# realphongha/UDP-Pose

Hardware: AMD Instinct MI355X
Metric: images/sec HRNet-W32 256x192 (infer+decode) (higher is better)
Workload: dtype f16x2 (split fp16 hi+lo operands = 22 bits, 3 fp16 MFMAs per product, fp32 accumulate); 1 GPU; w32 256x192 f16x2 inference, batch=64 per GPU, flip-test on, DARK decode (forward on 2N images + flip fuse + udp_decode_gaussian); global_batch=64, parallelism=replicas x1 (no data-path collective), weights=seeded synthetic, BN stats calibrated (tests/golden/bn_calib_w32_gaussian.npz)

## Files before the change

udp-pose_amd/csrc/conv_ws.hip:

```cpp
#include "conv_dev.h"

namespace udp {

#ifndef UDP_WS_LATE_RES
#define UDP_WS_LATE_RES 1
#endif
#ifndef UDP_WS_FAST_EPI
#define UDP_WS_FAST_EPI 1
#endif
#ifndef UDP_WS_FAST_ADDR
#define UDP_WS_FAST_ADDR 1
#endif
#ifdef UDP_OLD_SWZ
#undef UDP_WS_FAST_ADDR
#define UDP_WS_FAST_ADDR 0
#endif
#ifndef UDP_WS_INC_STEP
#define UDP_WS_INC_STEP 1
#endif
#if !UDP_WS_FAST_ADDR
#undef UDP_WS_INC_STEP
#define UDP_WS_INC_STEP 0
#endif
template <int NB>
struct ResH2 {
  u32x4 hi[NB / 2], lo[NB / 2];
};
template <int NB>
__device__ __forceinline__ void load_res_h2(ResH2<NB>& o, __amdgpu_buffer_rsrc_t r, unsigned voff, unsigned lo_off) {
#pragma unroll
  for (int h = 0; h < NB / 2; ++h) {
    o.hi[h] = __builtin_amdgcn_raw_buffer_load_b128(r, voff + 16 * h, 0, UDP_H2_RES_AUX);
    o.lo[h] = __builtin_amdgcn_raw_buffer_load_b128(r, voff + lo_off + 16 * h, 0, UDP_H2_RES_AUX);
  }
}
template <int NB>
__device__ __forceinline__ void add_res_h2(f32x4 (&v)[NB], const ResH2<NB>& o) {
#pragma unroll
  for (int h = 0; h < NB / 2; ++h) {
#if UDP_WS_FAST_EPI
    h2_add8_fast(v[2 * h], v[2 * h + 1], o.hi[h], o.lo[h]);
#else
    h2_add8(v[2 * h], v[2 * h + 1], __builtin_bit_cast(f16x8, o.hi[h]), __builtin_bit_cast(f16x8, o.lo[h]));
#endif
  }
}

template <int KS, int STRIDE, int PB, int CP, bool NCHW, bool OUT2 = false, int HS = 0, bool NUP = true, bool XP = false>
__device__ __forceinline__ void conv_ws_body(const ConvParams& p, const int tile_id, const int cby, const int xpair = 0) {
  using T = H2;
  constexpr int CK = 32, ESZ = 2, NB = 2, NW = 4;
  constexpr int PAD = KS / 2, TAPS = KS * KS;
  extern __shared__ __attribute__((aligned(UDP_WS_INC_STEP ? 512 : 16))) unsigned char smem[];

  UDP_STAMP(0);
  const int tid = threadIdx.x;
  const int lane = tid & 63;
  const int wave = __builtin_amdgcn_readfirstlane(tid >> 6);
  const int li = lane & 15;
  const int kg = lane >> 4;
  const int cp = wave % CP, pg = wave / CP;

  int t = tile_id;
  const int tx = t % p.tiles_x;
  t /= p.tiles_x;
  const int ty = t % p.tiles_y;
  const int n0 = (t / p.tiles_y) * p.G;
  const int y0 = ty * p.R;
  const int x0 = tx * p.TW;

  const int IH = p.IH, IW = p.IW;
  const int npix_in = p.G * IH * IW;
  const int in_groups = (npix_in + 15) >> 4;
  const int in_bytes = in_groups * 16 * ROWB;
  const int stage_bytes = 2 * in_bytes;
  const int nchunks = (p.Cin + CK - 1) / CK;
  const bool ragged = (p.Cin % CK) != 0;
  const int RT = p.R * p.TW;
  const int M = p.G * RT;
  const unsigned inpb = (unsigned)p.in_pitch * ESZ * 2;
  const unsigned outpb = (unsigned)p.out_pitch * ESZ * 2, respb = (unsigned)p.res_pitch * ESZ * 2;
  const unsigned in_lo = (unsigned)p.in_pitch * ESZ;
  const unsigned out_lo = (unsigned)p.out_pitch * ESZ, res_lo = (unsigned)p.res_pitch * ESZ;

  const unsigned out_pix = (unsigned)p.N * p.Hout * p.Wout;
  const __amdgpu_buffer_rsrc_t r_in = __builtin_amdgcn_make_buffer_rsrc(
      const_cast<void*>(p.in), 0, (unsigned)p.N * p.Hin * p.Win * inpb, 0x00020000);
  const unsigned npairs = (unsigned)p.CoutPad >> 5;
  const __amdgpu_buffer_rsrc_t r_w = __builtin_amdgcn_make_buffer_rsrc(
      const_cast<void*>(p.wgt), 0, (unsigned)TAPS * nchunks * npairs * 4096u, 0x00020000);
#if UDP_WS_DBG & 32
  const bool dbg_nost = nchunks == 1;
#else
  constexpr bool dbg_nost = false;
#endif
#if UDP_WS_DBG & 64
  const bool dbg_nores = nchunks == 1;
#else
  constexpr bool dbg_nores = false;
#endif
  const __amdgpu_buffer_rsrc_t r_out = __builtin_amdgcn_make_buffer_rsrc(
      p.out, 0, (!p.out || dbg_nost) ? 0 : NCHW ? (out_pix + (unsigned)p.out_skip * p.Hout * p.Wout) * p.Cout * 4 : out_pix * outpb, 0x00020000);
  const __amdgpu_buffer_rsrc_t r_bias = __builtin_amdgcn_make_buffer_rsrc(
      const_cast<float*>(p.bias), 0, (unsigned)p.CoutPad * 4u, 0x00020000);
  const __amdgpu_buffer_rsrc_t r_res = __builtin_amdgcn_make_buffer_rsrc(
      const_cast<void*>(p.res), 0, (p.res && !dbg_nores) ? out_pix * respb : 0, 0x00020000);

  const int pair = XP ? xpair : cby * CP + cp;
  const int cwave = pair * 32;
  const int cbase = cwave + 8 * kg;
  const unsigned wvoff = (unsigned)lane * 16u;
  const unsigned wpair = (unsigned)pair * 4096u;
  constexpr int AD = UDP_WS_AD;
  f16x8 ah[AD][NB], al[AD][NB];
  const int nsteps = nchunks * TAPS;
  auto load_a_at = [&](unsigned soff, f16x8 (&h)[NB], f16x8 (&l)[NB]) __attribute__((always_inline)) {
#pragma unroll
    for (int nb = 0; nb < NB; ++nb) {
      h[nb] = __builtin_bit_cast(f16x8, __builtin_amdgcn_raw_buffer_load_b128(r_w, wvoff + 2048u * nb, soff, 0));
      l[nb] = __builtin_bit_cast(f16x8, __builtin_amdgcn_raw_buffer_load_b128(r_w, wvoff + 2048u * nb + 1024u, soff, 0));
    }
  };
  auto load_a = [&](int s, f16x8 (&h)[NB], f16x8 (&l)[NB]) __attribute__((always_inline)) {
    const int c = s / TAPS, tap = s - c * TAPS;
    load_a_at((unsigned)(tap * nchunks + c) * (npairs * 4096u) + wpair, h, l);
  };

#pragma unroll
  for (int k = 0; k < AD - 1; ++k) load_a(k < nsteps ? k : nsteps - 1, ah[k], al[k]);
  f32x4 bias[NB];
#pragma unroll
  for (int nb = 0; nb < NB; ++nb)
    bias[nb] = __builtin_bit_cast(f32x4, __builtin_amdgcn_raw_buffer_load_b128(r_bias, (unsigned)(cbase + 4 * nb) * 4u, 0, 0));

  const int srow = lane >> 2, spart = lane & 3;
  const int gy0 = y0 * STRIDE - PAD, gx0 = x0 * STRIDE - PAD;
  unsigned src_off[MAXG];
#pragma unroll
  for (int i = 0; i < MAXG; ++i) {
    unsigned off = kOobOff;
    if ((wave + NW * i) * 16 < npix_in) {
      const int row = (wave + NW * i) * 16 + srow;
      const int tmp = fdiv20(row, p.mIW);
      const int ix = row - (int)__umul24(tmp, IW);
      const int g = fdiv20(tmp, p.mIH);
      const int iy = tmp - (int)__umul24(g, IH);
      const int n = n0 + g, gy = gy0 + iy, gx = gx0 + ix;
      const bool ok = row < npix_in && n < p.N && (unsigned)gy < (unsigned)p.Hin && (unsigned)gx < (unsigned)p.Win;
      const unsigned pix = __umul24(__umul24(n, p.Hin) + gy, p.Win) + gx;
      off = ok ? pix * inpb + p.in_coff * ESZ + ((spart ^ swz<T>(row)) << 4) : kOobOff;
    }
    src_off[i] = off;
  }
  auto stage = [&](int c, unsigned char* sb) __attribute__((always_inline)) {
    const unsigned coff = (unsigned)c * (CK * ESZ);
    const bool cut = ragged && c == nchunks - 1;
    const int parts_left = (p.Cin - c * CK) / 8;
#pragma unroll
    for (int i = 0; i < MAXG; ++i) {
      const int gidx = wave + NW * i;
      if (gidx < in_groups) {
        unsigned off = src_off[i] + coff;
        if (cut && (spart ^ swz<T>(gidx * 16 + srow)) >= parts_left) off = kOobOff;
        blds16(r_in, off, sb + gidx * (16 * ROWB));
        blds16(r_in, off + in_lo, sb + in_bytes + gidx * (16 * ROWB));
      }
    }
  };

  UDP_STAMP(1);
  stage(0, smem);

  int prow[PB], opix[PB], ocrd[NCHW || NUP ? PB : 1];
#pragma unroll
  for (int i = 0; i < PB; ++i) {
    const int m0 = (pg * PB + i) * 16 + li;
    const int m = m0 < M ? m0 : M - 1;
    const int g = fdiv20(m, p.mRT);
    const int rem = m - (int)__umul24(g, RT);
    const int r = fdiv20(rem, p.mTW);
    const int x = rem - (int)__umul24(r, p.TW);
    prow[i] = (int)__umul24(__umul24(g, IH) + r * STRIDE, IW) + x * STRIDE;
#if UDP_WS_FAST_ADDR
    prow[i] = prow[i] * ROWB + (kg << 4);
#endif
    const int n = n0 + g, y = y0 + r, xo = x0 + x;
    const bool ok = m0 < M && n < p.N && y < p.Hout && xo < p.Wout && (NCHW || cbase < p.Cout);
    const unsigned pix = __umul24(__umul24(n, p.Hout) + y, p.Wout) + xo;
    opix[i] = ok ? (int)pix : -1;
    if constexpr (NCHW || NUP) ocrd[i] = ok ? (y | (xo << 10) | (n << 20)) : -1;
  }

  const float winv = __builtin_ldexpf(1.f, -p.wexp);
  f32x4 acc[PB][NB];
#pragma unroll
  for (int i = 0; i < PB; ++i)
#pragma unroll
    for (int nb = 0; nb < NB; ++nb) acc[i][nb] = f32x4{0.f, 0.f, 0.f, 0.f};

  constexpr bool LATE = UDP_WS_LATE_RES && KS == 3 && STRIDE == 1 && !NCHW && AD == 3;
  constexpr int NR = NCHW ? 0 : PB * NB;
  ResH2<NB> rres[NCHW ? 1 : PB];
  constexpr int RSPLIT = LATE && PB > 6 ? PB / 2 : PB;
  auto load_res = [&](auto I0, auto I1) __attribute__((always_inline)) {
    __builtin_amdgcn_sched_barrier(0);
    asm volatile("" ::: "memory");
#pragma unroll
    for (int i = decltype(I0)::value; i < (NCHW ? 0 : decltype(I1)::value); ++i)
      load_res_h2(rres[i], r_res, opix[i] >= 0 ? (unsigned)opix[i] * respb + (p.res_coff + cbase) * ESZ : kOobOff, res_lo);
    asm volatile("" ::: "memory");
    __builtin_amdgcn_sched_barrier(0);
  };
  if constexpr (!LATE) load_res(std::integral_constant<int, 0>{}, std::integral_constant<int, PB>{});

  UDP_STAMP(2);
  int c = 0, tap = 0;
  const unsigned char* sb = smem;
  constexpr bool INC = UDP_WS_INC_STEP && LATE;
  using lds_u8 = const __attribute__((address_space(3))) unsigned char*;
  using lds_f16x8 = const __attribute__((address_space(3))) f16x8*;
  [[maybe_unused]] const unsigned lds0 = INC ? (unsigned)(size_t)(lds_u8)smem : 0u;
  [[maybe_unused]] const unsigned a_tap = (unsigned)nchunks * (npairs * 4096u);
  [[maybe_unused]] unsigned a_next = (unsigned)(AD - 1) * a_tap + wpair;
  [[maybe_unused]] int dy = 0;
  [[maybe_unused]] unsigned row_off = 0, sb_off = lds0;
  auto step = [&](auto BUFC, auto TAILC, int s) __attribute__((always_inline)) {
    constexpr int BUF = decltype(BUFC)::value, TAIL = decltype(TAILC)::value;
#if !(UDP_WS_DBG & 1)
    if constexpr (!LATE)
      load_a(s + AD - 1 < nsteps ? s + AD - 1 : nsteps - 1, ah[(BUF + AD - 1) % AD], al[(BUF + AD - 1) % AD]);
    else if constexpr (TAIL <= 0) {
      if constexpr (INC) {
        load_a_at(a_next, ah[(BUF + AD - 1) % AD], al[(BUF + AD - 1) % AD]);
        a_next += (BUF == 0 && dy == KS - 1) ? npairs * 4096u - (unsigned)(TAPS - 1) * a_tap : a_tap;
      } else {
        load_a(s + AD - 1, ah[(BUF + AD - 1) % AD], al[(BUF + AD - 1) % AD]);
      }
    }
#endif
    if constexpr (TAIL == 0) load_res(std::integral_constant<int, 0>{}, std::integral_constant<int, RSPLIT>{});
    if constexpr (TAIL == 1 && RSPLIT < PB) load_res(std::integral_constant<int, RSPLIT>{}, std::integral_constant<int, PB>{});
    if (TAIL < 0 && (INC ? BUF == 0 && dy == 0 : tap == 0)) {
      if (c == 1) UDP_STAMP(9);
      if (c == 2) UDP_STAMP(11);
      if (c == 4) UDP_STAMP(13);
      bool refill = false;
      if constexpr (STRIDE == 2 || OUT2) refill = p.sbuf && c > 0;
      if (refill) {
        __syncthreads();
        stage(c, smem);
        asm volatile("s_waitcnt vmcnt(0)" ::: "memory");
        __syncthreads();
        sb = smem;
        if constexpr (INC) sb_off = lds0;
      } else {
        if (s == 0)
          asm volatile("s_waitcnt vmcnt(%0)" ::"n"(2 * NB + (LATE ? 0 : NR)) : "memory");
        else
          asm volatile("s_waitcnt vmcnt(%0)" ::"n"(2 * NB) : "memory");
        if (s == 0) UDP_STAMP(3);
        __syncthreads();
        if (s == 0) UDP_STAMP(4);
        if (c == 1) UDP_STAMP(10);
        if (c == 2) UDP_STAMP(12);
        if (c == 4) UDP_STAMP(14);
#if !(UDP_WS_DBG & 4)
        if (c + 1 < nchunks && !((STRIDE == 2 || OUT2) && p.sbuf)) stage(c + 1, smem + ((c + 1) & 1) * stage_bytes);
#endif
        sb = smem + (c & 1) * stage_bytes;
        if constexpr (INC) sb_off = lds0 + (unsigned)((c & 1) * stage_bytes);
      }
    }
    f16x8 a2[NB];
#pragma unroll
    for (int nb = 0; nb < NB; ++nb) a2[nb] = ah[BUF][nb] * (_Float16)0x1p-11f;
    const int tap_rows = KS == 1 ? 0 : TAIL >= 0 ? (KS - 1) * IW + TAIL : (tap / KS) * IW + tap % KS;
    f16x8 xh[3], xl[3];
#if UDP_WS_FAST_ADDR
    const unsigned tap_off = INC ? sb_off + row_off + (unsigned)(BUF * ROWB) : (unsigned)(sb - smem) + (unsigned)tap_rows * ROWB;
    auto load_b = [&](int i, f16x8& h, f16x8& l) __attribute__((always_inline)) {
      const unsigned rb = (unsigned)prow[i] + tap_off;
      const unsigned a = __builtin_amdgcn_bitop3_b32(rb >> 3, rb, 32u, 0x6c);
      if constexpr (INC) {
        h = *reinterpret_cast<lds_f16x8>((size_t)a);
        l = *reinterpret_cast<lds_f16x8>((size_t)(a + (unsigned)in_bytes));
      } else {
        const unsigned char* q = smem + a;
        h = *reinterpret_cast<const f16x8*>(q);
        l = *reinterpret_cast<const f16x8*>(q + in_bytes);
      }
    };
#else
    auto load_b = [&](int i, f16x8& h, f16x8& l) __attribute__((always_inline)) {
      const int row = prow[i] + tap_rows;
      const unsigned char* q = sb + row * ROWB + ((kg ^ swz<T>(row)) << 4);
      h = *reinterpret_cast<const f16x8*>(q);
      l = *reinterpret_cast<const f16x8*>(q + in_bytes);
    };
#endif
    load_b(0, xh[0], xl[0]);
    if (PB > 1) load_b(1, xh[1], xl[1]);
#pragma unroll
    for (int i = 0; i < PB; ++i) {
#if !(UDP_WS_DBG & 2)
      if (i + 2 < PB) load_b(i + 2, xh[(i + 2) % 3], xl[(i + 2) % 3]);
#endif
      __builtin_amdgcn_sched_barrier(0);
#if UDP_WS_DBG & 16
      acc[i][0] = __builtin_amdgcn_mfma_f32_16x16x32_f16(ah[BUF][0] + al[BUF][1] + a2[0] + a2[1], xh[i % 3] + xl[i % 3], acc[i][0], 0, 0, 0);
#else
#pragma unroll
      for (int nb = 0; nb < NB; ++nb) acc[i][nb] = __builtin_amdgcn_mfma_f32_16x16x32_f16(ah[BUF][nb], xh[i % 3], acc[i][nb], 0, 0, 0);
#pragma unroll
      for (int nb = 0; nb < NB; ++nb) acc[i][nb] = __builtin_amdgcn_mfma_f32_16x16x32_f16(al[BUF][nb], xh[i % 3], acc[i][nb], 0, 0, 0);
#pragma unroll
      for (int nb = 0; nb < NB; ++nb) acc[i][nb] = __builtin_amdgcn_mfma_f32_16x16x32_f16(a2[nb], xl[i % 3], acc[i][nb], 0, 0, 0);
#endif
    }
    if constexpr (TAIL < 0) {
      if constexpr (INC) {
        if constexpr (BUF == KS - 1) {
          ++dy;
          row_off += (unsigned)IW * ROWB;
          if (dy == KS) {
            dy = 0;
            row_off = 0;
            ++c;
          }
        }
      } else if (++tap == TAPS) {
        tap = 0;
        ++c;
      }
    }
  };
  constexpr std::integral_constant<int, -1> LOOP{};
  if constexpr (LATE) {
    for (int s = 0; s < nsteps - AD; s += AD) {
      step(std::integral_constant<int, 0>{}, LOOP, s);
      step(std::integral_constant<int, 1>{}, LOOP, s + 1);
      step(std::integral_constant<int, 2>{}, LOOP, s + 2);
    }
    step(std::integral_constant<int, 0>{}, std::integral_constant<int, 0>{}, nsteps - 3);
    step(std::integral_constant<int, 1>{}, std::integral_constant<int, 1>{}, nsteps - 2);
    step(std::integral_constant<int, 2>{}, std::integral_constant<int, 2>{}, nsteps - 1);
  } else {
    for (int s = 0; s < nsteps; s += AD) {
      step(std::integral_constant<int, 0>{}, LOOP, s);
      if (s + 1 < nsteps) step(std::integral_constant<int, 1>{}, LOOP, s + 1);
      if (s + 2 < nsteps) step(std::integral_constant<int, 2>{}, LOOP, s + 2);
      if constexpr (AD > 3) if (s + 3 < nsteps) step(std::integral_constant<int, 3>{}, LOOP, s + 3);
      if constexpr (AD > 4) if (s + 4 < nsteps) step(std::integral_constant<int, 4>{}, LOOP, s + 4);
      if constexpr (AD > 5) if (s + 5 < nsteps) step(std::integral_constant<int, 5>{}, LOOP, s + 5);
    }
  }
  UDP_STAMP(5);
#pragma unroll
  for (int i = 0; i < PB; ++i) {
#pragma unroll
    for (int nb = 0; nb < NB; ++nb)
#pragma unroll
      for (int q = 0; q < 4; ++q) acc[i][nb][q] = __builtin_fmaf(acc[i][nb][q], winv, bias[nb][q]);
    if constexpr (!NCHW) add_res_h2(acc[i], rres[i]);
  }

#if UDP_WS_FAST_EPI
  [[maybe_unused]] const float relu_lim = p.relu ? 0.f : __builtin_nanf("");
#endif
#pragma unroll
  for (int i = 0; i < PB; ++i) {
    f32x4 v[NB];
#pragma unroll
    for (int nb = 0; nb < NB; ++nb) v[nb] = acc[i][nb];
    if constexpr (NCHW) {
      const int crd = ocrd[i];
      const int y = crd & 1023, xo = (crd >> 10) & 1023, n = crd >> 20;
      const unsigned hw = __umul24(p.Hout, p.Wout);
      const int no = n >= p.flip_from ? n + p.out_skip : n;
      const unsigned base = __umul24(__umul24(__umul24(no, p.Cout), p.Hout) + y, p.Wout) + xo;
#pragma unroll
      for (int nb = 0; nb < NB; ++nb)
#pragma unroll
        for (int q = 0; q < 4; ++q) {
          const int cc = cbase + 4 * nb + q;
          float f = v[nb][q];
          if (p.relu) f = f > 0.f ? f : 0.f;
          const unsigned off = (crd >= 0 && cc < p.Cout) ? (base + cc * hw) * 4u : kOobOff;
          __builtin_amdgcn_raw_buffer_store_b32(__builtin_bit_cast(unsigned, f), r_out, off, 0, 0);
        }
    } else {
      const unsigned ooff = opix[i] >= 0 ? (unsigned)opix[i] * outpb + (p.out_coff + cbase) * ESZ : kOobOff;
      if (NUP && p.nup) {
        const int crd = ocrd[NUP ? i : 0];
        const int y = crd & 1023, xo = (crd >> 10) & 1023, n = crd >> 20;
#pragma unroll
        for (int u = 0; u < 3; ++u) {
          if (u < p.nup) {
            const int sh = p.up_shift[u];
            const long up_pix = ((long)(n * (p.Hout >> sh) + (y >> sh)) * (p.Wout >> sh) + (xo >> sh));
            if (crd >= 0)
              add_vec<T, NB>(v, reinterpret_cast<const unsigned char*>(p.up[u]) + (up_pix * p.Cout * 2 + cbase) * ESZ, p.Cout * ESZ);
          }
        }
      }
#if UDP_WS_FAST_EPI
      unsigned mag;
      if constexpr (HS) {
#pragma unroll
        for (int nb = 0; nb < NB; ++nb)
#pragma unroll
          for (int q = 0; q < 4; ++q) v[nb][q] = act_hs<HS>(v[nb][q]);
        mag = h2_mag8<false>(0u, v[0], v[1]);
      } else {
        relu8_fast(v[0], v[1], relu_lim);
        mag = p.relu ? h2_mag8<true>(0u, v[0], v[1]) : h2_mag8<false>(0u, v[0], v[1]);
      }
      h2_range_check_bits(mag);
      u32x4 shi, slo;
      h2_split8_fast(v[0], v[1], shi, slo);
      __builtin_amdgcn_raw_buffer_store_b128(shi, r_out, ooff, 0, UDP_H2_STORE_AUX);
      __builtin_amdgcn_raw_buffer_store_b128(slo, r_out, ooff + out_lo, 0, UDP_H2_STORE_AUX);
#else
      if constexpr (HS) {
#pragma unroll
        for (int nb = 0; nb < NB; ++nb)
#pragma unroll
          for (int q = 0; q < 4; ++q) v[nb][q] = act_hs<HS>(v[nb][q]);
      } else
      if (p.relu) {
#pragma unroll
        for (int nb = 0; nb < NB; ++nb)
#pragma unroll
          for (int q = 0; q < 4; ++q) v[nb][q] = v[nb][q] > 0.f ? v[nb][q] : 0.f;
      }
      store_vec_buf<T, NB>(r_out, ooff, out_lo, v);
#endif
      if (OUT2 && p.nout2) {
        f16x8 sh, sl;
        h2_split8(v[0], v[1], sh, sl);
        f32x4 vr[NB];
#pragma unroll
        for (int q = 0; q < 4; ++q) {
          vr[0][q] = (float)sh[q] + (float)sl[q] * kLoInv;
          vr[1][q] = (float)sh[4 + q] + (float)sl[4 + q] * kLoInv;
        }
#pragma unroll
        for (int u = 0; u < 2; ++u) {
          if (u < p.nout2 && opix[i] >= 0) {
            const size_t px = (size_t)opix[i];
            const _Float16* a = reinterpret_cast<const _Float16*>(p.add2[u]) + px * (2 * (size_t)p.add2_pitch[u]) + p.add2_coff[u] + cbase;
            const f16x8 ah8 = *reinterpret_cast<const f16x8*>(a), al8 = *reinterpret_cast<const f16x8*>(a + p.add2_pitch[u]);
            f32x4 w[NB];
#pragma unroll
            for (int q = 0; q < 4; ++q) {
              w[0][q] = ((float)ah8[q] + (float)al8[q] * kLoInv) + vr[0][q];
              w[1][q] = ((float)ah8[4 + q] + (float)al8[4 + q] * kLoInv) + vr[1][q];
            }
            f16x8 oh, ol;
            h2_split8(w[0], w[1], oh, ol);
            _Float16* o2 = reinterpret_cast<_Float16*>(p.out2[u]) + px * (2 * (size_t)p.out2_pitch[u]) + p.out2_coff[u] + cbase;
            *reinterpret_cast<f16x8*>(o2) = oh;
            *reinterpret_cast<f16x8*>(o2 + p.out2_pitch[u]) = ol;
          }
        }
      }
    }
  }
  UDP_STAMP(6);
#ifdef UDP_STAMPS
  asm volatile("s_waitcnt vmcnt(0)" ::: "memory");
  UDP_STAMP(7);
#endif
}

__host__ __device__ __forceinline__ void ws_decode(unsigned b, unsigned ntiles, unsigned nc, int& tile, int& cby) {
  if (nc == 1) {
    tile = (int)b;
    cby = 0;
    return;
  }
  const unsigned full = (ntiles >> 3) * 8u * nc;
  unsigned base = 0, width = 8, r = b;
  if (b < full) {
    const unsigned g = b / (8u * nc);
    r = b - g * 8u * nc;
    base = g * 8u;
  } else {
    r = b - full;
    base = (ntiles >> 3) * 8u;
    width = ntiles & 7u;
  }
  const unsigned c = r / width;
  cby = (int)c;
  tile = (int)(base + r - c * width);
}

template <int KS, int STRIDE, int PB, int CP, bool NCHW>
__global__ __launch_bounds__(256, 2) void conv_ws_h2_kernel(const ConvParams p) {
  int tile, cby;
  ws_decode(blockIdx.x + gridDim.x * blockIdx.y, gridDim.x, gridDim.y, tile, cby);
  conv_ws_body<KS, STRIDE, PB, CP, NCHW, KS == 3 && STRIDE == 1 && !NCHW>(p, tile, cby);
}

template <int PB, int CP, int ACT>
__global__ __launch_bounds__(256, 2) void conv_ws_hs_kernel(const ConvParams p) {
  int tile, cby;
  ws_decode(blockIdx.x + gridDim.x * blockIdx.y, gridDim.x, gridDim.y, tile, cby);
  conv_ws_body<1, 1, PB, CP, false, false, ACT>(p, tile, cby);
}

#ifndef UDP_WS_MPB
#define UDP_WS_MPB 6
#define UDP_WS_MOCC 2
#endif
constexpr int kWsCode8 = 8;
constexpr bool kWsHave8 = UDP_WS_MPB == 6 && UDP_WS_LATE_RES && UDP_WS_AD == 3;
template <int KS>
__global__ __launch_bounds__(256, UDP_WS_MOCC) void conv_ws_multi(const ConvMulti m) {
  const unsigned b = blockIdx.x;
  int j, tile, cby;
  int code;
  const unsigned e = __builtin_amdgcn_readfirstlane(m.tab[(b >> 3) < (unsigned)kMultiTab ? (b >> 3) : 0u]);
  if (m.tab_n) {
    j = (int)(e & 3u);
    code = 1 << ((e >> 2) & 3u);
    cby = (int)((e >> 4) & 63u);
    tile = (int)((e >> 10) + (b & 7u));
  } else {
    int sg = 0;
#pragma unroll
    for (int k = 1; k < kMultiSegs; ++k) sg += b >= m.seg_start[k];
    j = __builtin_amdgcn_readfirstlane(m.seg_mem[sg]);
    const unsigned r = __builtin_amdgcn_readfirstlane(b - m.seg_start[sg] + m.seg_first[sg]);
    ws_decode(r, m.tiles[j], m.ncby[j], tile, cby);
    tile = __builtin_amdgcn_readfirstlane(tile);
    cby = __builtin_amdgcn_readfirstlane(cby);
    code = m.code[j];
  }
  if constexpr (KS == 3 && kWsHave8) {
    if (code == kWsCode8) {
      conv_ws_body<KS, 1, 8, 1, false, false, 0, false>(m.p[j], tile, (int)cby);
      return;
    }
  }
  switch (code) {
    case 1: conv_ws_body<KS, 1, UDP_WS_MPB, 1, false>(m.p[j], tile, (int)cby); break;
    case 2: conv_ws_body<KS, 1, UDP_WS_MPB, 2, false>(m.p[j], tile, (int)cby); break;
    default: conv_ws_body<KS, 1, UDP_WS_MPB, 4, false>(m.p[j], tile, (int)cby); break;
  }
}

__global__ __launch_bounds__(256, 2) void conv_ws_pb8_kernel(const ConvParams p) {
  conv_ws_body<3, 1, 8, 1, false, false, 0, false>(p, (int)blockIdx.x, (int)blockIdx.y);
}

__device__ __forceinline__ void s2x_side(const ConvParams& p, const ConvParams& f, const int tile_id) {
  extern __shared__ __attribute__((aligned(16))) unsigned char smem[];
  int t = tile_id;
  const int tx = t % p.tiles_x;
  t /= p.tiles_x;
  const int ty = t % p.tiles_y;
  const int n0 = (t / p.tiles_y) * p.G;
  const int IH = p.IH, IW = p.IW;
  const int in_bytes = ((p.G * IH * IW + 15) >> 4) * 16 * ROWB;
  const int PW = 2 * p.TW, PHW = 2 * p.R * PW;
  const int gy0 = 2 * ty * p.R, gx0 = 2 * tx * p.TW;
  const int items = p.G * PHW * 4;
  const unsigned outpb = (unsigned)f.out_pitch * 4u, out_lo = (unsigned)f.out_pitch * 2u;
  const __amdgpu_buffer_rsrc_t r_out = __builtin_amdgcn_make_buffer_rsrc(f.out, 0, (unsigned)f.N * f.Hout * f.Wout * outpb, 0x00020000);
  for (int it = threadIdx.x; it < items; it += 256) {
    const int part = it & 3, pp = it >> 2;
    const int g = fdiv20(pp, f.mRT);
    const int rem = pp - g * PHW;
    const int r = fdiv20(rem, f.mTW);
    const int x = rem - r * PW;
    const int n = n0 + g, gy = gy0 + r, gx = gx0 + x;
    if (n >= p.N || gy >= p.Hin || gx >= p.Win) continue;
    const int row = (g * IH + r + 1) * IW + x + 1;
    const unsigned char* q = smem + row * ROWB + ((part ^ swz<H2>(row)) << 4);
    const f16x8 hi = *reinterpret_cast<const f16x8*>(q), lo = *reinterpret_cast<const f16x8*>(q + in_bytes);
    f32x4 v[2];
#pragma unroll
    for (int k = 0; k < 4; ++k) {
      v[0][k] = (float)hi[k] + (float)lo[k] * kLoInv;
      v[1][k] = (float)hi[4 + k] + (float)lo[4 + k] * kLoInv;
    }
    const int c = 8 * part;
#pragma unroll
    for (int u = 0; u < 3; ++u) {
      if (u < f.nup) {
        const int sh = f.up_shift[u];
        const size_t up_pix = ((size_t)(n * (f.Hout >> sh) + (gy >> sh)) * (f.Wout >> sh) + (gx >> sh));
        add_vec<H2, 2>(v, reinterpret_cast<const unsigned char*>(f.up[u]) + (up_pix * f.Cout * 2 + c) * 2, f.Cout * 2);
      }
    }
    if (f.relu) {
#pragma unroll
      for (int k = 0; k < 4; ++k) {
        v[0][k] = v[0][k] > 0.f ? v[0][k] : 0.f;
        v[1][k] = v[1][k] > 0.f ? v[1][k] : 0.f;
      }
    }
    const unsigned pix = __umul24(__umul24(n, p.Hin) + gy, p.Win) + gx;
    store_vec_buf<H2, 2>(r_out, pix * outpb + (unsigned)(f.out_coff + c) * 2u, out_lo, v);
  }
}

template <int PB, int CP>
__global__ __launch_bounds__(256, 2) void conv_ws_s2x_kernel(const ConvShare m) {
  const int slot = __builtin_amdgcn_readfirstlane((int)(threadIdx.x >> 6)) % CP;
  const int r = __builtin_amdgcn_readfirstlane((int)((m.route >> (8 * slot)) & 255u));
  const int lp = __builtin_amdgcn_readfirstlane((int)((m.lpair >> (8 * slot)) & 255u));
  conv_ws_body<3, 2, PB, CP, false, false, 0, true, true>(m.p[r], (int)blockIdx.x, 0, lp);
  if (m.side.out) s2x_side(m.p[0], m.side, (int)blockIdx.x);
}

template <int KS, int STRIDE, int PB, int CP, bool NCHW>
static int describe_ws_one(const ConvParams& p, size_t lds, Launch* out) {
  static bool attr_set = false;
  const void* kern = reinterpret_cast<const void*>(&conv_ws_h2_kernel<KS, STRIDE, PB, CP, NCHW>);
  if (!attr_set) {
    UDP_HIP_CHECK(hipFuncSetAttribute(kern, hipFuncAttributeMaxDynamicSharedMemorySize, 160 * 1024));
    attr_set = true;
  }
  out->fn = kern;
  out->grid = dim3(p.ntiles, p.CoutPad / (CP * 32));
  out->block = dim3(256);
  out->lds = (unsigned)lds;
  out->p = p;
  return UDP_OK;
}
template <int KS, int STRIDE, bool NCHW>
static int describe_ws_pb(const ConvParams& p, int pb, int cp, size_t lds, Launch* out) {
#define UDP_WS(B, C) \
  if (pb == B && cp == C) return describe_ws_one<KS, STRIDE, B, C, NCHW>(p, lds, out);
  UDP_WS(2, 1) UDP_WS(3, 1) UDP_WS(4, 1) UDP_WS(6, 1) UDP_WS(2, 2) UDP_WS(3, 2) UDP_WS(4, 2) UDP_WS(6, 2)
  UDP_WS(2, 4) UDP_WS(3, 4) UDP_WS(4, 4) UDP_WS(6, 4)
#undef UDP_WS
  return 1;
}
static int describe_ws_pb8(const ConvParams& p, size_t lds, Launch* out) {
  static bool attr_set = false;
  const void* kern = reinterpret_cast<const void*>(&conv_ws_pb8_kernel);
  if (!attr_set) {
    UDP_HIP_CHECK(hipFuncSetAttribute(kern, hipFuncAttributeMaxDynamicSharedMemorySize, 160 * 1024));
    attr_set = true;
  }
  out->fn = kern;
  out->grid = dim3(p.ntiles, p.CoutPad / 32);
  out->block = dim3(256);
  out->lds = (unsigned)lds;
  out->p = p;
  return UDP_OK;
}
template <int PB, int CP, int ACT>
static int describe_ws_hs_one(const ConvParams& p, size_t lds, Launch* out) {
  static bool attr_set = false;
  const void* kern = reinterpret_cast<const void*>(&conv_ws_hs_kernel<PB, CP, ACT>);
  if (!attr_set) {
    UDP_HIP_CHECK(hipFuncSetAttribute(kern, hipFuncAttributeMaxDynamicSharedMemorySize, 160 * 1024));
    attr_set = true;
  }
  out->fn = kern;
  out->grid = dim3(p.ntiles, p.CoutPad / (CP * 32));
  out->block = dim3(256);
  out->lds = (unsigned)lds;
  out->p = p;
  return UDP_OK;
}
static int describe_ws_hs(const ConvParams& p, int pb, int cp, size_t lds, Launch* out) {
#define UDP_WS(B, C) \
  if (pb == B && cp == C) return p.relu == UDP_ACT_SILU ? describe_ws_hs_one<B, C, UDP_ACT_SILU>(p, lds, out) : describe_ws_hs_one<B, C, UDP_ACT_HSWISH>(p, lds, out);
  UDP_WS(2, 1) UDP_WS(3, 1) UDP_WS(4, 1) UDP_WS(6, 1) UDP_WS(2, 2) UDP_WS(3, 2) UDP_WS(4, 2) UDP_WS(6, 2)
  UDP_WS(2, 4) UDP_WS(3, 4) UDP_WS(4, 4) UDP_WS(6, 4)
#undef UDP_WS
  return 1;
}
static bool ws_tile(const ConvParams& p, int ks, int stride, int cp, int pb, WsTile* t, bool own_launch) {
  const int pg = 4 / cp;
  const int maxM = 16 * pb * pg;
  bool have = false;
  double best_util = 0.0;
  for (int split = 1; split <= 4 || !have; ++split) {
    if (split > 8) break;
    const int TW = ceil_div(p.Wout, split);
    if (TW > 64 || TW > maxM || (have && TW < 8)) continue;
    int maxR = maxM / TW;
    if (maxR > p.Hout) maxR = p.Hout;
    int R = largest_divisor_leq(p.Hout, maxR);
    if (R * 2 <= maxR) R = maxR;
    int G = 1;
    if (R == p.Hout && TW == p.Wout) {
      G = maxM / (R * TW);
      if (G > p.N) G = p.N;
      if (G < 1) G = 1;
    }
    auto npix = [&](int g, int r) { return g * ((r - 1) * stride + ks) * ((TW - 1) * stride + ks); };
    while (npix(G, R) > MAXG * 64 && G > 1) --G;
    while (npix(G, R) > MAXG * 64 && R > 1) R = (R + 1) / 2;
    if (npix(G, R) > MAXG * 64) continue;
    int nstage = ceil_div(p.Cin, 32) > 1 ? 2 : 1;
    size_t lds = (size_t)((npix(G, R) + 15) / 16) * 16 * ROWB * 2 * nstage;
    static const int sbuf_mode = getenv("UDP_POSE_WS_SBUF") == nullptr ? 1 : atoi(getenv("UDP_POSE_WS_SBUF"));
    const bool sbuf_kernel = stride == 2 || (ks == 3 && own_launch && sbuf_mode != 2);
    const bool sbuf = sbuf_kernel && nstage == 2 && lds > 80 * 1024 && lds / 2 <= 80 * 1024 && sbuf_mode != 0;
    if (sbuf) {
      nstage = 1;
      lds /= 2;
    }
    if (lds > 160 * 1024) continue;
    if (pb == 8 && (G * R * TW != maxM || p.Hout % R || TW * split != p.Wout || lds > 80 * 1024)) continue;
    const int need = ceil_div(ceil_div(G * R * TW, 16), pg);
    if (need > pb) continue;
    const int pbe = need <= 2 ? 2 : need <= 3 ? 3 : need <= 4 ? 4 : need <= 6 ? 6 : 8;
    const int tiles = ceil_div(p.N, G) * ceil_div(p.Hout, R) * ceil_div(p.Wout, TW);
    const double util = (double)p.N * p.Hout * p.Wout / ((double)tiles * 16 * pbe * pg) *
                        ((double)G * R * TW * stride * stride / (double)npix(G, R));
    if (!have || util > best_util + 0.05) {
      have = true;
      best_util = util;
      t->cp = cp;
      t->pb = pbe;
      t->G = G;
      t->R = R;
      t->TW = TW;
      t->lds = lds;
      t->sbuf = sbuf ? 1 : 0;
      t->wgs = tiles * (p.CoutPad / (cp * 32));
    }
  }
  return have;
}

static long g_ws_fill_wgs = 512;
void ws_set_fill_wgs(long wgs) { g_ws_fill_wgs = wgs; }

int choose_conv_ws(ConvParams& p, int ks, int stride, bool grouped, WsTile* best_out) {
  if (p.relu >= UDP_ACT_HSWISH && (ks != 1 || stride != 1 || p.out_nchw_f32 || p.res || p.nup || p.nout2 || grouped))
    return fail(UDP_ERR_UNSUPPORTED, "hard-swish / SiLU (activation codes 2, 4): plain 1x1 stride-1 NHWC convs on their own launch only");
  if ((stride != 1 && stride != 2) || (ks != 3 && ks != 1) || (p.out_nchw_f32 && stride != 1))
    return fail(UDP_ERR_UNSUPPORTED, "fragment-major weights (wfmt 1): conv ks=%d stride=%d nchw_out=%d has no weight-stationary kernel",
                ks, stride, p.out_nchw_f32);
  auto knob = [](const char* name, long dflt) {
    const char* v = getenv(name);
    return v ? atol(v) : dflt;
  };
  const int pairs = p.CoutPad / 32;
  const int force_cp = (int)knob("UDP_POSE_WS_CP", 0), force_pb = (int)knob("UDP_POSE_WS_PB", 0);
  const long min_wgs = grouped ? 0 : knob("UDP_POSE_WS_MINWGS", g_ws_fill_wgs);
  const bool offer8 = kWsHave8 && grouped && ks == 3 && stride == 1 && pairs % 2 == 1 && !p.out_nchw_f32 && !p.nout2 && !p.nup &&
                      knob("UDP_POSE_WS_PB8", 1) != 0;
  WsTile best{}, t{};
  bool have = false;
  for (int pb : {8, 6, 4, 3, 2}) {
    for (int cp : {4, 2, 1}) {
      if (pb == 8 && (!offer8 || cp != 1)) continue;
      if (pairs % cp || (force_cp && cp != force_cp) || (force_pb && pb != force_pb)) continue;
      if (grouped && stride == 1 && UDP_WS_MPB != 6 && pb != UDP_WS_MPB) continue;
      if (!ws_tile(p, ks, stride, cp, pb, &t, !grouped && !p.out_nchw_f32)) continue;
      const bool fills = t.wgs >= min_wgs, best_fills = have && best.wgs >= min_wgs;
      if (!have || (!best_fills && (fills || t.wgs > best.wgs))) {
        best = t;
        have = true;
      }
    }
  }
  if (!have) return fail(UDP_ERR_UNSUPPORTED, "weight-stationary conv: no tile for %dx%d C%d->%d", p.Hout, p.Wout, p.Cin, p.Cout);
  p.G = best.G;
  p.R = best.R;
  p.TW = best.TW;
  p.sbuf = best.sbuf;
  p.IH = (p.R - 1) * stride + ks;
  p.IW = (p.TW - 1) * stride + ks;
  p.tiles_x = ceil_div(p.Wout, p.TW);
  p.tiles_y = ceil_div(p.Hout, p.R);
  auto magic = [](int d) { return (unsigned)(((1u << 20) + (unsigned)d - 1) / (unsigned)d); };
  p.mIW = magic(p.IW);
  p.mIH = magic(p.IH);
  p.mRT = magic(p.R * p.TW);
  p.mTW = magic(p.TW);
  p.ntiles = ceil_div(p.N, p.G) * p.tiles_y * p.tiles_x;
  if (getenv("UDP_POSE_DEBUG_TILES"))
    fprintf(stderr, "ws conv k%d s%d %dx%d C%d->%d: G=%d R=%d TW=%d CP=%d PB=%d lds=%zu%s wgs=%d\n", ks, stride, p.Hout, p.Wout, p.Cin,
            p.Cout, p.G, p.R, p.TW, best.cp, best.pb, best.lds, best.sbuf ? " (one stage buffer)" : "", best.wgs);
  *best_out = best;
  return UDP_OK;
}

int describe_conv_ws(ConvParams p, int ks, int stride, Launch* out, bool grouped) {
  WsTile best{};
  if (const int crc = choose_conv_ws(p, ks, stride, grouped, &best)) return crc;
  int rc = 1;
  if (best.pb == 8) {
    rc = describe_ws_pb8(p, best.lds, out);
  } else
  if (ks == 3 && stride == 1 && !p.out_nchw_f32) rc = describe_ws_pb<3, 1, false>(p, best.pb, best.cp, best.lds, out);
  if (ks == 3 && stride == 1 && p.out_nchw_f32) rc = describe_ws_pb<3, 1, true>(p, best.pb, best.cp, best.lds, out);
  if (ks == 3 && stride == 2) rc = describe_ws_pb<3, 2, false>(p, best.pb, best.cp, best.lds, out);
  if (ks == 1 && stride == 1 && !p.out_nchw_f32)
    rc = p.relu >= UDP_ACT_HSWISH ? describe_ws_hs(p, best.pb, best.cp, best.lds, out) : describe_ws_pb<1, 1, false>(p, best.pb, best.cp, best.lds, out);
  if (ks == 1 && stride == 1 && p.out_nchw_f32) rc = describe_ws_pb<1, 1, true>(p, best.pb, best.cp, best.lds, out);
  if (ks == 1 && stride == 2) rc = describe_ws_pb<1, 2, false>(p, best.pb, best.cp, best.lds, out);
  if (rc == 1) return fail(UDP_ERR_UNSUPPORTED, "weight-stationary conv: no kernel for PB=%d CP=%d", best.pb, best.cp);
  if (rc == UDP_OK && p.nout2 && !(ks == 3 && stride == 1))
    return fail(UDP_ERR_UNSUPPORTED, "second outputs: 3x3 stride-1 convs only");
  if (rc == UDP_OK && grouped && (best.pb == UDP_WS_MPB || best.pb == 8) && stride == 1 && !p.nout2) {
    out->groupable = 300 + ks * 10 + (best.pb == 8 ? 8 : 6);
    out->ws_cp = best.cp;
  }
  return rc;
}

template <int PB, int CP>
static int describe_s2x_one(size_t lds, int ntiles, Launch* out) {
  static bool attr_set = false;
  const void* kern = reinterpret_cast<const void*>(&conv_ws_s2x_kernel<PB, CP>);
  if (!attr_set) {
    UDP_HIP_CHECK(hipFuncSetAttribute(kern, hipFuncAttributeMaxDynamicSharedMemorySize, 160 * 1024));
    attr_set = true;
  }
  out->fn = kern;
  out->grid = dim3(ntiles);
  out->block = dim3(256);
  out->lds = (unsigned)lds;
  return UDP_OK;
}

static bool choose_share_tile(const ConvParams& c0, int cp, WsTile* best) {
  ConvParams q = c0;
  q.Cout = q.CoutPad = cp * 32;
  const char* v = getenv("UDP_POSE_WS_MINWGS");
  const long min_wgs = v ? atol(v) : g_ws_fill_wgs;
  WsTile t{};
  bool have = false;
  for (int pb : {6, 4, 3, 2}) {
    if (!ws_tile(q, 3, 2, cp, pb, &t, false) || t.lds > 80 * 1024 || t.sbuf) continue;
    const bool fills = t.wgs >= min_wgs, best_fills = have && best->wgs >= min_wgs;
    if (!have || (!best_fills && (fills || t.wgs > best->wgs))) {
      *best = t;
      have = true;
    }
  }
  return have;
}

int describe_x0_share(const ConvParams* convs, int n, const ConvParams* fuse, const char* tag, Launch* out) {
  if (n < 1 || n > kShareRoutes) return 1;
  const ConvParams& c0 = convs[0];
  int pairs = 0;
  for (int j = 0; j < n; ++j) {
    const ConvParams& c = convs[j];
    if (c.Cin != 32 || c.wfmt != 1 || c.out_nchw_f32 || c.nout2 || c.in_stuff2 || c.bn_ws || c.relu > UDP_ACT_RELU || !c.out || c.in != c0.in ||
        c.in_pitch != c0.in_pitch || c.in_coff != c0.in_coff || c.N != c0.N || c.Hin != c0.Hin || c.Win != c0.Win || c.Hout != c0.Hout ||
        c.Wout != c0.Wout || c.CoutPad % 32 || c.CoutPad / 32 > 4)
      return 1;
    pairs += c.CoutPad / 32;
  }
  if (pairs > 4 || n + (fuse ? 1 : 0) < 2) return 1;
  if (fuse && (fuse->in != c0.in || fuse->in_pitch != c0.in_pitch || fuse->in_coff != c0.in_coff || fuse->Cout != 32 || fuse->N != c0.N ||
               fuse->Hout != c0.Hin || fuse->Wout != c0.Win || fuse->res || !fuse->out || fuse->relu > UDP_ACT_RELU || fuse->out_pitch % 8 ||
               fuse->out_coff % 8 || (size_t)fuse->N * fuse->Hout * fuse->Wout * fuse->out_pitch * 4 >= 0x7FFF0000u))
    return 1;
  const int cp = pairs <= 2 ? 2 : 4;
  WsTile best{};
  if (!choose_share_tile(c0, cp, &best)) return 1;
  auto m = std::make_shared<ConvShare>();
  memset(m.get(), 0, sizeof(ConvShare));
  auto magic = [](int d) { return (unsigned)(((1u << 20) + (unsigned)d - 1) / (unsigned)d); };
  int ntiles = 0;
  for (int j = 0; j < n; ++j) {
    ConvParams& p = m->p[j];
    p = convs[j];
    p.G = best.G;
    p.R = best.R;
    p.TW = best.TW;
    p.sbuf = 0;
    p.IH = (p.R - 1) * 2 + 3;
    p.IW = (p.TW - 1) * 2 + 3;
    p.tiles_x = ceil_div(p.Wout, p.TW);
    p.tiles_y = ceil_div(p.Hout, p.R);
    p.mIW = magic(p.IW);
    p.mIH = magic(p.IH);
    p.mRT = magic(p.R * p.TW);
    p.mTW = magic(p.TW);
    p.ntiles = ntiles = ceil_div(p.N, p.G) * p.tiles_y * p.tiles_x;
  }
  for (int j = n; j < kShareRoutes; ++j) m->p[j] = m->p[0];
  int slot = 0;
  for (int j = 0; j < n; ++j)
    for (int lp = 0; lp < convs[j].CoutPad / 32; ++lp, ++slot) {
      m->route |= (unsigned)j << (8 * slot);
      m->lpair |= (unsigned)lp << (8 * slot);
    }
  for (; slot < cp; ++slot) m->lpair |= 255u << (8 * slot);
  if (fuse) {
    m->side = *fuse;
    m->side.mRT = magic(4 * best.R * best.TW);
    m->side.mTW = magic(2 * best.TW);
  }
  int rc = 1;
#define UDP_S2X(B, C) \
  if (best.pb == B && cp == C) rc = describe_s2x_one<B, C>(best.lds, ntiles, out);
  UDP_S2X(2, 2) UDP_S2X(3, 2) UDP_S2X(4, 2) UDP_S2X(6, 2) UDP_S2X(2, 4) UDP_S2X(3, 4) UDP_S2X(4, 4) UDP_S2X(6, 4)
#undef UDP_S2X
  if (rc) return rc;
  out->groupable = 0;
  out->ws_cp = 0;
  out->pair = 0;
  out->p = m->p[0];
  out->share = m;
  if (getenv("UDP_POSE_DEBUG_TILES")) {
    char routes[64] = "";
    for (int j = 0; j < n; ++j) snprintf(routes + strlen(routes), sizeof(routes) - strlen(routes), "%s%d", j ? "," : "", convs[j].Cout);
    fprintf(stderr, "x0 share %dx%d C32: %s pairs=%d routes=[%s] fuse0=%d G=%d R=%d TW=%d CP=%d PB=%d lds=%zu wgs=%d\n", c0.Hin, c0.Win, tag ? tag : "",
            pairs, routes, fuse ? 1 : 0, best.G, best.R, best.TW, cp, best.pb, best.lds, ntiles);
  }
  return UDP_OK;
}

static void ws_order(ConvMulti* m, int n) {
  struct Seg {
    unsigned start, first, cnt;
    int mem;
  };
  unsigned cnt_of[4];
  unsigned total = 0;
  for (int j = 0; j < n; ++j) {
    cnt_of[j] = (j + 1 < n ? m->start[j + 1] : m->start[4]) - m->start[j];
    total += cnt_of[j];
  }
  const char* mode = getenv("UDP_POSE_WS_ORDER");
  const bool lpt = mode && strcmp(mode, "lpt") == 0;
  const unsigned bias = getenv("UDP_POSE_WS_BIAS") ? (unsigned)atoi(getenv("UDP_POSE_WS_BIAS")) : 125u;
  auto build = [&](unsigned g) {
    std::vector<Seg> segs;
    unsigned lo[4] = {0, 0, 0, 0};
    unsigned at = 0;
    auto take = [&](int j, unsigned cnt) {
      if (cnt > cnt_of[j] - lo[j]) cnt = cnt_of[j] - lo[j];
      if (!cnt) return;
      if (!segs.empty() && segs.back().mem == j && segs.back().first + segs.back().cnt == lo[j])
        segs.back().cnt += cnt;
      else
        segs.push_back({at, lo[j], cnt, j});
      lo[j] += cnt;
      at += cnt;
    };
    if (!lpt) {
      const unsigned nb = cnt_of[n - 1];
      const unsigned na = total - nb;
      unsigned ta = 0, tb = 0;
      while (ta < na && tb < nb) {
        if ((unsigned long long)ta * nb * 100ull <= (unsigned long long)tb * na * bias) {
          int j = 0;
          while (lo[j] == cnt_of[j]) ++j;
          const unsigned c = cnt_of[j] - lo[j] < g ? cnt_of[j] - lo[j] : g;
          take(j, c);
          ta += c;
        } else {
          const unsigned c = nb - tb < g ? nb - tb : g;
          take(n - 1, c);
          tb += c;
        }
      }
    }
    for (int j = 0; j < n; ++j) take(j, cnt_of[j] - lo[j]);
    return segs;
  };
  unsigned g = getenv("UDP_POSE_WS_G") ? (unsigned)atoi(getenv("UDP_POSE_WS_G")) : 32u;
  if (g < 8 || g % 8) g = 32;
  std::vector<Seg> segs = build(g);
  m->tab_n = 0;
  bool ok = total % 8 == 0 && total / 8 <= (unsigned)kMultiTab && getenv("UDP_POSE_WS_NOTAB") == nullptr;
  for (int j = 0; j < n && ok; ++j)
    ok = m->tiles[j] % 8 == 0 && m->ncby[j] <= 64 && m->tiles[j] < (1u << 22) && (m->code[j] == 1 || m->code[j] == 2 || m->code[j] == 4 || m->code[j] == kWsCode8);
  for (size_t k = 0; k < segs.size() && ok; ++k) ok = segs[k].start % 8 == 0 && segs[k].first % 8 == 0;
  if (ok) {
    for (const Seg& sg : segs) {
      const int j = sg.mem;
      for (unsigned b = sg.start; b < sg.start + sg.cnt; b += 8) {
        int tile, cby;
        ws_decode(b - sg.start + sg.first, m->tiles[j], m->ncby[j], tile, cby);
        const unsigned cl = m->code[j] == 1 ? 0u : m->code[j] == 2 ? 1u : m->code[j] == 4 ? 2u : 3u;
        m->tab[b >> 3] = (unsigned)j | (cl << 2) | ((unsigned)cby << 4) | ((unsigned)tile << 10);
      }
    }
    m->tab_n = total / 8;
  }
  while (segs.size() > (size_t)kMultiSegs) {
    g += 8;
    segs = build(g);
  }
  for (int k = 0; k < kMultiSegs; ++k) {
    const bool have = (size_t)k < segs.size();
    m->seg_start[k] = have ? segs[k].start : 0xFFFFFFFFu;
    m->seg_first[k] = have ? segs[k].first : 0;
    m->seg_mem[k] = have ? segs[k].mem : 0;
  }
}

extern "C" int udp_debug_multi_order(const unsigned* tiles, const unsigned* ncby, const int* code, int n, unsigned cap,
                                     unsigned* out_member, unsigned* out_tile, unsigned* out_cby, int* used_table) {
  if (!tiles || !ncby || !code || n < 1 || n > 4 || !out_member || !out_tile || !out_cby) return -1;
  static ConvMulti m;
  memset(&m, 0, sizeof(m));
  unsigned total = 0;
  for (int j = 0; j < n; ++j) {
    m.start[j] = total;
    m.tiles[j] = tiles[j];
    m.ncby[j] = ncby[j];
    m.code[j] = code[j];
    total += tiles[j] * ncby[j];
  }
  for (int j = n; j < 5; ++j) m.start[j] = j < 4 ? 0xFFFFFFFFu : total;
  m.start[4] = total;
  for (int j = n; j < 4; ++j) m.tiles[j] = m.ncby[j] = 1;
  if (total > cap) return -1;
  ws_order(&m, n);
  if (used_table) *used_table = m.tab_n != 0;
  for (unsigned b = 0; b < total; ++b) {
    int j, tile, cby;
    if (m.tab_n) {
      const unsigned e = m.tab[b >> 3];
      j = (int)(e & 3u);
      if ((1 << ((e >> 2) & 3u)) != m.code[j]) return -1;
      cby = (int)((e >> 4) & 63u);
      tile = (int)((e >> 10) + (b & 7u));
    } else {
      int sg = 0;
      for (int k = 1; k < kMultiSegs; ++k) sg += b >= m.seg_start[k];
      j = m.seg_mem[sg];
      ws_decode(b - m.seg_start[sg] + m.seg_first[sg], m.tiles[j], m.ncby[j], tile, cby);
    }
    out_member[b] = (unsigned)j;
    out_tile[b] = (unsigned)tile;
    out_cby[b] = (unsigned)cby;
  }
  return (int)total;
}

int describe_ws_multi(const Launch* members, int n, ConvMulti* m, Launch* out) {
  static bool ws_attr_set = false;
  const void* wk[2] = {reinterpret_cast<const void*>(&conv_ws_multi<3>), reinterpret_cast<const void*>(&conv_ws_multi<1>)};
  if (!ws_attr_set) {
    for (const void* k : wk) UDP_HIP_CHECK(hipFuncSetAttribute(k, hipFuncAttributeMaxDynamicSharedMemorySize, 160 * 1024));
    ws_attr_set = true;
  }
  memset(m, 0, sizeof(*m));
  unsigned total = 0, lds = 0;
  for (int j = 0; j < n; ++j) {
    if (members[j].groupable / 10 != members[0].groupable / 10) return fail(UDP_ERR_ARG, "describe_multi: mixed weight-stationary members");
    m->p[j] = members[j].p;
    m->start[j] = total;
    m->tiles[j] = members[j].grid.x;
    m->ncby[j] = members[j].grid.y;
    m->code[j] = members[j].groupable % 10 == 8 ? kWsCode8 : members[j].ws_cp;
    total += members[j].grid.x * members[j].grid.y;
    if (members[j].lds > lds) lds = members[j].lds;
  }
  for (int j = n; j < 5; ++j) m->start[j] = j < 4 ? 0xFFFFFFFFu : total;
  for (int j = n; j < 4; ++j) m->tiles[j] = m->ncby[j] = 1;
  ws_order(m, n);
  if (getenv("UDP_POSE_DEBUG_TILES")) {
    char codes[64] = "";
    for (int j = 0; j < n; ++j) snprintf(codes + strlen(codes), sizeof(codes) - strlen(codes), "%s%d", j ? "," : "", m->code[j]);
    fprintf(stderr, "ws multi k%d: members=%d wgs=%u codes=[%s] dispatch=%s\n", members[0].groupable / 10 % 10, n, total, codes,
            m->tab_n ? "table" : "search");
  }
  out->fn = wk[members[0].groupable / 10 % 10 == 3 ? 0 : 1];
  out->grid = dim3(total);
  out->block = dim3(256);
  out->lds = lds;
  out->groupable = 0;
  return UDP_OK;
}

#ifdef UDP_STAMPS
int ws_set_stamps(unsigned long long* dev_buf) {
  UDP_HIP_CHECK(hipMemcpyToSymbol(HIP_SYMBOL(g_stamps), &dev_buf, sizeof(dev_buf)));
  return UDP_OK;
}
extern "C" int udp_debug_set_stamps_ws(unsigned long long* dev_buf) { return ws_set_stamps(dev_buf); }
#endif

template <int NCH, int PB, int RD, bool LDSW>
__global__ __launch_bounds__(LDSW ? 512 : 256) __attribute__((amdgpu_waves_per_eu(2))) void conv_chain_kernel(const ConvParams p) {
  using T = H2;
  constexpr int ESZ = 2, NB = 2, Q = 2;
  constexpr int NWAVES = LDSW ? 8 : 4;
  constexpr int AD = LDSW ? 2 : 3;
  extern __shared__ __attribute__((aligned(16))) unsigned char smem[];
  const int lane = threadIdx.x & 63, wave = __builtin_amdgcn_readfirstlane(threadIdx.x >> 6);
  const int li = lane & 15, kg = lane >> 4;
  const unsigned npix = (unsigned)p.N * p.Hout * p.Wout;
  constexpr int NP = 8;
  const int cout2 = p.up_shift[0];
// ... 414 lines not shown
```

Baseline: 9141 images/s.

## Specialise PB=8 conv arm to constant tile shape and add row-walk stride-2 path

Adds a compile-time specialised path for the 8-block weight-stationary 3x3 conv with a fixed 612-row input tile, one channel chunk and one image per tile. Pixel addressing is computed with shifts instead of magic-number divisions, and the 9-step loop is fully unrolled. The host side now rejects any tile that does not match these constants. It also extends the incremental row-offset addressing and late A-load path to 3x3 stride-2 convs. The aim is to cut scalar and vector address arithmetic and loop overhead, at the cost of a narrower, hard-coded shape contract.

Result: no change. 9139 images/s (-0.0%).

```diff
diff --git a/udp-pose_amd/csrc/conv_ws.hip b/udp-pose_amd/csrc/conv_ws.hip
--- a/udp-pose_amd/csrc/conv_ws.hip
+++ b/udp-pose_amd/csrc/conv_ws.hip
@@ -22,6 +22,21 @@
 #undef UDP_WS_INC_STEP
 #define UDP_WS_INC_STEP 0
 #endif
+#ifndef UDP_WS_INC_S2
+#define UDP_WS_INC_S2 1
+#endif
+#if !UDP_WS_INC_STEP
+#undef UDP_WS_INC_S2
+#define UDP_WS_INC_S2 0
+#endif
+#ifndef UDP_WS_PB8_CONST
+#define UDP_WS_PB8_CONST 1
+#endif
+#if !UDP_WS_INC_STEP
+#undef UDP_WS_PB8_CONST
+#define UDP_WS_PB8_CONST 0
+#endif
+constexpr int kWs8Rows = 612, kWs8Groups = (kWs8Rows + 15) / 16;
 template <int NB>
 struct ResH2 {
   u32x4 hi[NB / 2], lo[NB / 2];
@@ -51,6 +66,7 @@
   using T = H2;
   constexpr int CK = 32, ESZ = 2, NB = 2, NW = 4;
   constexpr int PAD = KS / 2, TAPS = KS * KS;
+  constexpr bool C8 = UDP_WS_PB8_CONST && PB == 8 && CP == 1 && KS == 3 && STRIDE == 1 && !NCHW && !OUT2 && !NUP;
   extern __shared__ __attribute__((aligned(UDP_WS_INC_STEP ? 512 : 16))) unsigned char smem[];
 
   UDP_STAMP(0);
@@ -65,19 +81,19 @@
   const int tx = t % p.tiles_x;
   t /= p.tiles_x;
   const int ty = t % p.tiles_y;
-  const int n0 = (t / p.tiles_y) * p.G;
+  const int n0 = C8 ? t / p.tiles_y : (t / p.tiles_y) * p.G;
   const int y0 = ty * p.R;
   const int x0 = tx * p.TW;
 
   const int IH = p.IH, IW = p.IW;
-  const int npix_in = p.G * IH * IW;
+  const int npix_in = C8 ? kWs8Rows : p.G * IH * IW;
   const int in_groups = (npix_in + 15) >> 4;
   const int in_bytes = in_groups * 16 * ROWB;
   const int stage_bytes = 2 * in_bytes;
-  const int nchunks = (p.Cin + CK - 1) / CK;
+  const int nchunks = C8 ? 1 : (p.Cin + CK - 1) / CK;
   const bool ragged = (p.Cin % CK) != 0;
-  const int RT = p.R * p.TW;
-  const int M = p.G * RT;
+  const int RT = C8 ? 16 * PB * NW : p.R * p.TW;
+  const int M = C8 ? RT : p.G * RT;
   const unsigned inpb = (unsigned)p.in_pitch * ESZ * 2;
   const unsigned outpb = (unsigned)p.out_pitch * ESZ * 2, respb = (unsigned)p.res_pitch * ESZ * 2;
   const unsigned in_lo = (unsigned)p.in_pitch * ESZ;
@@ -143,7 +159,7 @@
       const int row = (wave + NW * i) * 16 + srow;
       const int tmp = fdiv20(row, p.mIW);
       const int ix = row - (int)__umul24(tmp, IW);
-      const int g = fdiv20(tmp, p.mIH);
+      const int g = C8 ? 0 : fdiv20(tmp, p.mIH);
       const int iy = tmp - (int)__umul24(g, IH);
       const int n = n0 + g, gy = gy0 + iy, gx = gx0 + ix;
       const bool ok = row < npix_in && n < p.N && (unsigned)gy < (unsigned)p.Hin && (unsigned)gx < (unsigned)p.Win;
@@ -172,6 +188,19 @@
   stage(0, smem);
 
   int prow[PB], opix[PB], ocrd[NCHW || NUP ? PB : 1];
+  if constexpr (C8) {
+    const int wsh = p.TW >> 5;
+    const int lane_row = li * ROWB + (kg << 4);
+    const bool lane_ok = n0 < p.N && cbase < p.Cout;
+#pragma unroll
+    for (int i = 0; i < PB; ++i) {
+      const int b = pg * PB + i;
+      const int r = b >> wsh, xu = (b << 4) & (p.TW - 1);
+      prow[i] = (r * IW + xu) * ROWB + lane_row;
+      const int pix = ((n0 * p.Hout + y0 + r) * p.Wout + x0 + xu) + li;
+      opix[i] = lane_ok ? pix : -1;
+    }
+  } else {
 #pragma unroll
   for (int i = 0; i < PB; ++i) {
     const int m0 = (pg * PB + i) * 16 + li;
@@ -190,6 +219,7 @@
     opix[i] = ok ? (int)pix : -1;
     if constexpr (NCHW || NUP) ocrd[i] = ok ? (y | (xo << 10) | (n << 20)) : -1;
   }
+  }
 
   const float winv = __builtin_ldexpf(1.f, -p.wexp);
   f32x4 acc[PB][NB];
@@ -216,7 +246,9 @@
   UDP_STAMP(2);
   int c = 0, tap = 0;
   const unsigned char* sb = smem;
-  constexpr bool INC = UDP_WS_INC_STEP && LATE;
+  constexpr bool S2R = UDP_WS_INC_S2 && KS == 3 && STRIDE == 2 && !NCHW && AD == 3;
+  constexpr bool ROWL = LATE || S2R;
+  constexpr bool INC = (UDP_WS_INC_STEP && LATE) || S2R;
   using lds_u8 = const __attribute__((address_space(3))) unsigned char*;
   using lds_f16x8 = const __attribute__((address_space(3))) f16x8*;
   [[maybe_unused]] const unsigned lds0 = INC ? (unsigned)(size_t)(lds_u8)smem : 0u;
@@ -227,7 +259,7 @@
   auto step = [&](auto BUFC, auto TAILC, int s) __attribute__((always_inline)) {
     constexpr int BUF = decltype(BUFC)::value, TAIL = decltype(TAILC)::value;
 #if !(UDP_WS_DBG & 1)
-    if constexpr (!LATE)
+    if constexpr (!ROWL)
       load_a(s + AD - 1 < nsteps ? s + AD - 1 : nsteps - 1, ah[(BUF + AD - 1) % AD], al[(BUF + AD - 1) % AD]);
     else if constexpr (TAIL <= 0) {
       if constexpr (INC) {
@@ -238,8 +270,8 @@
       }
     }
 #endif
-    if constexpr (TAIL == 0) load_res(std::integral_constant<int, 0>{}, std::integral_constant<int, RSPLIT>{});
-    if constexpr (TAIL == 1 && RSPLIT < PB) load_res(std::integral_constant<int, RSPLIT>{}, std::integral_constant<int, PB>{});
+    if constexpr (LATE && TAIL == 0) load_res(std::integral_constant<int, 0>{}, std::integral_constant<int, RSPLIT>{});
+    if constexpr (LATE && TAIL == 1 && RSPLIT < PB) load_res(std::integral_constant<int, RSPLIT>{}, std::integral_constant<int, PB>{});
     if (TAIL < 0 && (INC ? BUF == 0 && dy == 0 : tap == 0)) {
       if (c == 1) UDP_STAMP(9);
       if (c == 2) UDP_STAMP(11);
@@ -335,7 +367,18 @@
     }
   };
   constexpr std::integral_constant<int, -1> LOOP{};
-  if constexpr (LATE) {
+  if constexpr (C8) {
+    static_assert(LATE && INC, "the 8-block arm is a LATE body");
+    step(std::integral_constant<int, 0>{}, LOOP, 0);
+    step(std::integral_constant<int, 1>{}, LOOP, 1);
+    step(std::integral_constant<int, 2>{}, LOOP, 2);
+    step(std::integral_constant<int, 0>{}, LOOP, 3);
+    step(std::integral_constant<int, 1>{}, LOOP, 4);
+    step(std::integral_constant<int, 2>{}, LOOP, 5);
+    step(std::integral_constant<int, 0>{}, std::integral_constant<int, 0>{}, 6);
+    step(std::integral_constant<int, 1>{}, std::integral_constant<int, 1>{}, 7);
+    step(std::integral_constant<int, 2>{}, std::integral_constant<int, 2>{}, 8);
+  } else if constexpr (ROWL) {
     for (int s = 0; s < nsteps - AD; s += AD) {
       step(std::integral_constant<int, 0>{}, LOOP, s);
       step(std::integral_constant<int, 1>{}, LOOP, s + 1);
@@ -792,6 +835,10 @@
   if (const int crc = choose_conv_ws(p, ks, stride, grouped, &best)) return crc;
   int rc = 1;
   if (best.pb == 8) {
+    if (!(p.G == 1 && p.R * p.TW == 512 && (p.TW == 16 || p.TW == 32) && p.IH * p.IW == kWs8Rows && p.Hout % p.R == 0 && p.Wout % p.TW == 0 &&
+          p.Cin <= 32 && !p.sbuf && best.lds == (size_t)kWs8Groups * 16 * ROWB * 2 && ks == 3 && stride == 1))
+      return fail(UDP_ERR_UNSUPPORTED, "weight-stationary conv: the 8-block arm got a tile it is not built for (G=%d R=%d TW=%d Cin=%d lds=%zu)",
+                  p.G, p.R, p.TW, p.Cin, best.lds);
     rc = describe_ws_pb8(p, best.lds, out);
   } else
   if (ks == 3 && stride == 1 && !p.out_nchw_f32) rc = describe_ws_pb<3, 1, false>(p, best.pb, best.cp, best.lds, out);
```
